# neherlab/pangraph

Measured on AMD Instinct MI355X. Metric: aligned Gbp/s in `pangraph build` (bases handed to the aligner per second, all merges, all self-merge rounds), higher is better.
Workload: dtype u8

## Files before the change

pangraph_amd/csrc/pga_chain.hip:

```cpp
#include "pga_common.h"
#include "pga_sort_exact.h"
#include "pga_sort_wave.h"
#include "pga_wave.h"
#include "pga_pipeline.h"
#include "pga_wg_sort.h"
#include <rocprim/rocprim.hpp>
#include <cstdio>

namespace pga {

struct ChainParams {
	int32_t max_dist, max_dist_inner, bw, max_skip, cap, min_cnt, min_sc;
	float pen_gap, pen_skip;
};

struct __attribute__((aligned(16))) CNode {
	double pri;
	int32_t y;
	int32_t c[2];
	int32_t s;
	uint32_t size;
	int32_t bal;
};

// ... 158 lines not shown
		if (root < 0) return -1;
		for (p = root; p >= 0;) { c = cmp(lo_y, lo_i, p); path[0][plen[0]] = p, pc[0][plen[0]++] = (int8_t)c; if (c < 0) p = nd[p].c[0]; else if (c > 0) p = nd[p].c[1]; else break; }
		for (p = root; p >= 0;) { c = cmp(hi_y, hi_i, p); path[1][plen[1]] = p, pc[1][plen[1]++] = (int8_t)c; if (c < 0) p = nd[p].c[0]; else if (c > 0) p = nd[p].c[1]; else break; }
		for (i = 0; i < plen[0] && i < plen[1]; ++i)
			if (path[0][i] == path[1][i] && pc[0][i] <= 0 && pc[1][i] >= 0) break;
		if (i == plen[0] || i == plen[1]) return -1;
		lca = i, mn = path[0][lca];
		for (i = lca + 1; i < plen[0]; ++i) if (pc[0][i] <= 0) {
			int32_t u = path[0][i], r = nd[u].c[1];
			if (nd[u].pri < nd[mn].pri) mn = u;
			if (r >= 0 && nd[nd[r].s].pri < nd[mn].pri) mn = nd[r].s;
		}
		for (i = lca + 1; i < plen[1]; ++i) if (pc[1][i] >= 0) {
			int32_t u = path[1][i], l = nd[u].c[0];
			if (nd[u].pri < nd[mn].pri) mn = u;
			if (l >= 0 && nd[nd[l].s].pri < nd[mn].pri) mn = nd[l].s;
		}
		return mn;
	}
};

struct Iter { int32_t stack[CMAXD]; int top; };


#define CF_WI 1024
#define CF_MAXIN 256

__device__ __forceinline__ int32_t score_pair32(int32_t xi, int32_t yi, int32_t xj, int32_t yj, int32_t span_j, float pen_gap, float pen_skip, int32_t *exact, int32_t *width)
{
	const int32_t dq = yi - yj, dr = xi - xj;
	const int32_t dd = dr > dq ? dr - dq : dq - dr;
	const int32_t dg = dr < dq ? dr : dq;
	int32_t sc = span_j < dg ? span_j : dg;
	*width = dd;
	if (exact) *exact = (dd == 0 && dg <= span_j);
	if (dd || dq > span_j) {
		float lin_pen = __fadd_rn(__fmul_rn(pen_gap, (float)dd), __fmul_rn(pen_skip, (float)dg));
		float log_pen = dd >= 1 ? mg_log2((float)(dd + 1)) : 0.0f;
		sc -= (int)__fadd_rn(lin_pen, __fmul_rn(.5f, log_pen));
	}
	return sc;
}

struct __attribute__((aligned(8))) CfEnt { int32_t y, x; };
__device__ __forceinline__ double cf_pri(int32_t f, int32_t x, int32_t y, float pen_gap) { return -((double)f + 0.5 * (double)pen_gap * (double)(x + y)); }

#define CF_CLK() (PROF == 2 ? (long long)clock64() : 0LL)
template <int CF_W, int PROF>
__global__ __launch_bounds__(64)
void k_chain_fast(const u128 *__restrict__ a, const uint64_t *__restrict__ seg_start, const uint32_t *__restrict__ seg_order, uint32_t n_seg,
                  uint64_t n_total, const uint64_t *__restrict__ q_aoff, int n_seq, ChainParams P,
                  int32_t *__restrict__ f, int32_t *__restrict__ pp, uint32_t *__restrict__ seg_flag, const uint32_t *__restrict__ only_flagged, unsigned long long *__restrict__ prof)
{
	constexpr int CF_M = CF_W - 1;
	__shared__ CfEnt r_e[CF_W];
	__shared__ int32_t r_f[CF_W];
	__shared__ uint8_t s_sp[CF_W];
	__shared__ int32_t r_p[CF_WI], r_t[CF_WI];
	__shared__ int32_t s_sc[CF_WI], s_j[CF_WI];
	__shared__ uint8_t s_fl[CF_WI];
	const int lane = threadIdx.x;
	const uint32_t sidx = blockIdx.x;
	if (sidx >= n_seg) return;
	const uint32_t sg = seg_order[sidx];
	if (only_flagged && !only_flagged[sg]) return;
	const uint64_t b = seg_start[sg], e = sg + 1 < n_seg ? seg_start[sg + 1] : n_total;
	const int32_t n = (int32_t)(e - b);
	const u128 *A = a + b;
	int32_t *F = f + b, *PP = pp + b;
	int qlo = 0, qhi = n_seq;
	while (qlo < qhi) { int m = (qlo + qhi) >> 1; if (q_aoff[m + 1] <= b) qlo = m + 1; else qhi = m; }
	const bool seg_is_query_start = (q_aoff[qlo] == b);
	int32_t max_dist = P.max_dist, max_dist_inner = P.max_dist_inner;
	if (max_dist < P.bw) max_dist = P.bw;
	if (max_dist_inner <= 0 || max_dist_inner >= max_dist) max_dist_inner = 0;
	for (int k = lane; k < CF_WI; k += 64) r_t[k] = -1;
	int32_t st = 0, st_in = 0, i0 = 0;
	bool bail = false; int why = 0;
	double sm_pri = 1e300; int32_t sm_arg = -1, sm_blk = -1, sm_ymin = 0, sm_ymax = 0;
	double p_floor = 1e300, p_last = 1e300;
	const int32_t FS_NONE = -(1 << 30);
	int32_t fs_floor = FS_NONE, fs_last = FS_NONE, sm_fs = FS_NONE;
	const bool shortcut_ok = P.cap >= CF_W;
	const unsigned long long c0 = wall_clock64();
	unsigned long long n_scan = 0, n_inner = 0, n_incand = 0, n_slow = 0, n_pev = 0, n_py = 0;
	unsigned long long n_stretch = 0, n_chunk = 0, n_skipstop = 0, n_sum = 0, n_sumscan = 0;
	long long tk_scan = 0, tk_red = 0, tk_best = 0, tk_inner = 0, tk_store = 0;
	u128 nxtv; nxtv.x = 0, nxtv.y = 0;
	if (lane < n) nxtv = A[lane];
	for (int32_t blk = 0; blk < n && !bail; blk += 64) {
		const int32_t bx = (int32_t)nxtv.x, by = (int32_t)nxtv.y, bsp = (int32_t)(nxtv.y >> 32 & 0xff);
		int32_t bf = 0;
		if (blk + lane < n) { const int32_t s = (blk + lane) & CF_M; r_e[s].x = bx; r_e[s].y = by; s_sp[s] = (uint8_t)bsp; }
		if (blk + 64 + lane < n) nxtv = A[blk + 64 + lane];
		__builtin_amdgcn_fence(__ATOMIC_SEQ_CST, "wavefront");
		{
			const int32_t xb = __builtin_amdgcn_readlane(bx, 0);
			for (;;) {
				const int32_t j = st + lane;
				const bool keep = j >= i0 || !(xb - r_e[j & CF_M].x > max_dist);
				const unsigned long long m = __ballot(keep);
				if (m) { st += __ffsll((long long)m) - 1; break; }
				st += 64;
			}
			p_floor = wave_min_f64_key((lane < CF_W / 64 && sm_blk >= 0 && sm_blk + 64 > st) ? sm_pri : 1e300);
			fs_floor = wave_max_i32((lane < CF_W / 64 && sm_blk >= 0 && sm_blk + 64 > st) ? sm_fs : FS_NONE);
		}
		if (blk + 128 - st > CF_W) { bail = true; why = 1; break; }
		const int32_t blk_end = blk + 64 < n ? blk + 64 : n;
		for (int32_t i = blk; i < blk_end; ++i) {
			const int il = i - blk;
			const int32_t xi = __builtin_amdgcn_readlane(bx, il), yi = __builtin_amdgcn_readlane(by, il), q_span = __builtin_amdgcn_readlane(bsp, il);
			int32_t max_f = q_span, max_j = -1;
			if (shortcut_ok && il > 0 && i0 == i - 1 && p_last < p_floor) {
				const int32_t xpl = wave_shr1(bx, 0), ypl = wave_shr1(by, 0), spl = wave_shr1(bsp, 0);
				const int32_t dr = bx - xpl, dq = by - ypl;
				const int32_t f_l = __builtin_amdgcn_readlane(bf, il - 1) + (bx - __builtin_amdgcn_readlane(bx, il - 1));
				const bool c_ok = lane >= il && blk + lane < blk_end && dr > 0 && dr <= max_dist && dq == dr && dr <= spl && dr < max_dist && f_l > bsp;
				const unsigned long long m2 = __ballot(c_ok) >> il;
				const int R = ~m2 ? __ffsll((long long)~m2) - 1 : 64;
				if (R >= 2) {
					if (lane >= il && lane < il + R) { bf = f_l; r_f[(blk + lane) & CF_M] = f_l; r_p[(blk + lane) & (CF_WI - 1)] = blk + lane - 1; }
					__builtin_amdgcn_fence(__ATOMIC_SEQ_CST, "wavefront");
					const int la = il + R - 2, lb = il + R - 1;
					p_floor = cf_pri(__builtin_amdgcn_readlane(bf, la), __builtin_amdgcn_readlane(bx, la), __builtin_amdgcn_readlane(by, la), P.pen_gap);
					p_last = cf_pri(__builtin_amdgcn_readlane(bf, lb), __builtin_amdgcn_readlane(bx, lb), __builtin_amdgcn_readlane(by, lb), P.pen_gap);
					{
						const int32_t fsm = wave_max_i32((lane >= il && lane < il + R - 1) ? bf + bsp : FS_NONE);
						fs_floor = max(max(fs_floor, fs_last), fsm);
						fs_last = __builtin_amdgcn_readlane(bf, lb) + __builtin_amdgcn_readlane(bsp, lb);
					}
					if (PROF) { n_py += R; n_stretch += R; }
					i0 = i + R - 1;
					i += R - 1;
					continue;
				}
			}
			long long k0 = CF_CLK(), k1 = k0, k2 = k0;
			int32_t best_j = -1;
			bool shortcut = false;
			if (shortcut_ok && il > 0 && i0 == i - 1) {
				const int32_t xp = __builtin_amdgcn_readlane(bx, il - 1), yp = __builtin_amdgcn_readlane(by, il - 1);
				if (xp != xi && xi - xp <= max_dist && yp < yi && yp > yi - max_dist && p_last < p_floor) { shortcut = true; best_j = i - 1; i0 = i; if (PROF) ++n_py; }
			}
			if (il > 0 && p_last < p_floor) p_floor = p_last;
			if (!shortcut) {
			if (i0 < i) { const int32_t x0 = i0 >= blk ? __builtin_amdgcn_readlane(bx, i0 - blk) : r_e[i0 & CF_M].x; if (x0 != xi) i0 = i; }
			k0 = CF_CLK();
			for (;;) {
				const int32_t j = st + lane;
				const bool keep = j >= i0 || !(xi - r_e[j & CF_M].x > max_dist);
				const unsigned long long m = __ballot(keep);
				if (m) { st += __ffsll((long long)m) - 1; break; }
				st += 64;
			}
			double best = 1e300; bool tie = false;
			{
				const int32_t y_lo = yi - max_dist;
				auto scan64 = [&](int32_t j0, int32_t jend) {
					++n_scan;
					const int32_t j = j0 + lane;
					if (j >= st && j < jend) {
						const CfEnt ej = r_e[j & CF_M];
						const bool in = ej.y > y_lo && (ej.y < yi || (ej.y == yi && seg_is_query_start && j == 0));
						if (in) { const double pj = cf_pri(r_f[j & CF_M], ej.x, ej.y, P.pen_gap); if (pj < best) best = pj, best_j = j, tie = false; else if (pj == best) tie = true; }
					}
				};
				const int32_t S = blk < (i0 & ~63) ? blk : (i0 & ~63);
				bool part = false, took = false;
				if (lane < CF_W / 64 && sm_blk >= 0 && sm_blk + 64 > st && sm_blk + 64 <= S) {
					const bool none = sm_ymax <= y_lo || sm_ymin > yi || (sm_ymin == yi && !(seg_is_query_start && sm_blk == 0));
					if ((sm_blk >= st || sm_arg >= st) && sm_ymin > y_lo && sm_ymax < yi) { best = sm_pri; best_j = sm_arg < 0 ? sm_blk : sm_arg; tie = sm_arg < 0; took = true; }
					else if (!none) part = true;
				}
				unsigned long long pm = __ballot(part);
				if (PROF) { n_sum += __popcll(__ballot(took)); n_sumscan += __popcll(pm); }
				while (pm) {
					const int bsel = __ffsll((long long)pm) - 1;
					pm &= pm - 1;
					const int32_t bb = __builtin_amdgcn_readlane(sm_blk, bsel);
					scan64(bb, bb + 64);
				}
				if (i0 > blk) {
					++n_scan;
					const int32_t j = blk + lane;
					if (j >= st && j < i0) {
						const bool in = by > y_lo && (by < yi || (by == yi && seg_is_query_start && j == 0));
						if (in) { const double pj = cf_pri(bf, bx, by, P.pen_gap); if (pj < best) best = pj, best_j = j, tie = false; else if (pj == best) tie = true; }
					}
				} else for (int32_t tj = S > st ? S : st; tj < i0; tj += 64) scan64(tj, i0);
			}
			if (i0 - st > P.cap) { bail = true; why = 2; break; }
			k1 = CF_CLK();
			{
				const unsigned long long bits = (unsigned long long)__double_as_longlong(best);
				const unsigned long long key = (bits >> 63) ? ~bits : (bits | 0x8000000000000000ULL);
				const uint32_t khi = (uint32_t)(key >> 32), klo = (uint32_t)key;
				const uint32_t mhi = wave_min_u32(khi);
				const uint32_t mlo = wave_min_u32(khi == mhi ? klo : 0xffffffffu);
				const bool is_min = khi == mhi && klo == mlo;
				const unsigned long long who = __ballot(best_j >= 0 && is_min);
				if (who == 0) best_j = -1;
				else {
					if (__popcll(who) > 1 || __ballot(tie && is_min)) { bail = true; why = 3; break; }
					best_j = __builtin_amdgcn_readlane(best_j, __ffsll((long long)who) - 1);
				}
			}
			}
			k2 = CF_CLK();
			long long k3 = k2;
			if (best_j >= 0) {
				int32_t exact, width; const int32_t j = best_j;
				CfEnt ej; int32_t fj, spj;
				if (j >= blk) { const int jl = j - blk; ej.x = __builtin_amdgcn_readlane(bx, jl); ej.y = __builtin_amdgcn_readlane(by, jl); fj = __builtin_amdgcn_readlane(bf, jl); spj = __builtin_amdgcn_readlane(bsp, jl); }
				else { ej = r_e[j & CF_M]; fj = r_f[j & CF_M]; spj = s_sp[j & CF_M]; }
				int32_t sc = fj + score_pair32(xi, yi, ej.x, ej.y, spj, P.pen_gap, P.pen_skip, &exact, &width);
				if (width <= P.bw && sc > max_f) max_f = sc, max_j = j;
				k3 = CF_CLK();
				if (!exact && (j == i - 1 ? fs_floor : max(fs_floor, fs_last)) <= max_f) { exact = 1; if (PROF) ++n_pev; }
				if (!exact && max_dist_inner > 0 && yi > 0) {
					if (st_in < st) st_in = st;
					{
						const int32_t lo = i0 - (CF_MAXIN + 1);
						if (lo > st_in && xi - r_e[lo & CF_M].x > max_dist_inner) st_in = lo + 1;
					}
					for (;;) {
						const int32_t jj = st_in + lane;
						const bool keep = jj >= i0 || !(xi - r_e[jj & CF_M].x > max_dist_inner);
						const unsigned long long m = __ballot(keep);
						if (m) { st_in += __ffsll((long long)m) - 1; break; }
						st_in += 64;
					}
					if (st_in > i0) st_in = i0;
				}
				if (!exact && max_dist_inner > 0 && st_in < i0 && yi > 0) {
					const int32_t n_in = i0 - st_in;
					if (n_in > CF_WI) { bail = true; why = 4; break; }
					if (n_in > CF_MAXIN) {
						++n_inner; n_incand += n_in; if (PROF) ++n_chunk;
						auto cand = [&](int32_t jc, int32_t &sc, bool &ok) -> bool {
							const CfEnt ec = r_e[jc & CF_M];
							if (!(ec.y <= yi - 1 && ec.y >= yi - max_dist_inner)) { sc = 0; ok = false; return false; }
							int32_t wdt;
							sc = r_f[jc & CF_M] + score_pair32(xi, yi, ec.x, ec.y, s_sp[jc & CF_M], P.pen_gap, P.pen_skip, nullptr, &wdt);
							ok = wdt <= P.bw;
							return true;
						};
						bool unsorted = false;
						for (int32_t c0 = 0; c0 < n_in; c0 += 64) {
							const int32_t jc = i0 - 1 - (c0 + lane);
							if (jc >= st_in) {
								if (jc + 1 < i0 && r_e[(jc + 1) & CF_M].y < r_e[jc & CF_M].y) unsorted = true;
								int32_t sc; bool ok;
								if (cand(jc, sc, ok) && ok) { const int32_t pj = r_p[jc & (CF_WI - 1)]; if (pj >= st_in) r_t[pj & (CF_WI - 1)] = i; }
							}
						}
						__builtin_amdgcn_fence(__ATOMIC_SEQ_CST, "wavefront");
						const bool uns = __ballot(unsorted) != 0;
						int32_t n_slots = n_in;
						if (uns) {
							++n_slow;
							n_slots = 0;
							for (int32_t c0 = 0; c0 < n_in; c0 += 64) {
								const int32_t jc = i0 - 1 - (c0 + lane);
								int32_t sc = 0; bool ok = false;
								const bool val = jc >= st_in && cand(jc, sc, ok);
								n_slots += __popcll(__ballot(val));
								if (val) {
									const int32_t yc = r_e[jc & CF_M].y;
									int32_t rank = 0;
									for (int32_t jo = st_in; jo < i0; ++jo) {
										const int32_t yo = r_e[jo & CF_M].y;
										const bool vo = yo <= yi - 1 && yo >= yi - max_dist_inner;
										rank += (vo && (yo > yc || (yo == yc && jo > jc))) ? 1 : 0;
									}
									s_sc[rank] = sc; s_j[rank] = jc;
									s_fl[rank] = (uint8_t)((ok ? 1 : 0) | (r_t[jc & (CF_WI - 1)] == i ? 2 : 0));
								}
							}
							__builtin_amdgcn_fence(__ATOMIC_SEQ_CST, "wavefront");
						}
						int32_t n_skip = 0; bool stop = false;
						for (int32_t c0 = 0; c0 < n_slots && !stop; c0 += 64) {
							int32_t v_sc = 0, v_j = -1; bool v_ok = false, v_mk = false;
							if (uns) {
								const int32_t c = c0 + lane;
								if (c < n_slots) { const int32_t fl = s_fl[c]; v_ok = fl & 1; v_mk = (fl & 2) != 0; v_sc = s_sc[c]; v_j = s_j[c]; }
							} else {
								const int32_t jc = i0 - 1 - (c0 + lane);
								if (jc >= st_in) { v_j = jc; const bool val = cand(jc, v_sc, v_ok); v_mk = val && r_t[jc & (CF_WI - 1)] == i; }
							}
							const int32_t v = v_ok ? v_sc : INT32_MIN;
							const int32_t incl = wave_prefix_max_incl(v);
							int32_t excl = __builtin_amdgcn_update_dpp(max_f, incl, 0x138, 0xf, 0xf, false);
							if (excl < max_f) excl = max_f;
							const bool is_max = v_ok && v_sc > excl;
							const unsigned long long mx = __ballot(is_max), inc = __ballot(v_ok && !is_max && v_mk);
							unsigned long long rest = mx; int last = -1, pos = 0;
							for (;;) {
								const int c = rest ? __ffsll((long long)rest) - 1 : 64;
								const unsigned long long range = (c >= 64 ? ~0ULL : ((1ULL << c) - 1)) & ~((1ULL << pos) - 1);
								n_skip += __popcll(inc & range);
// ... 18 lines not shown
						if (jc >= st_in) {
							const CfEnt ec = r_e[jc & CF_M];
							if (jc + 1 < i0 && r_e[(jc + 1) & CF_M].y < ec.y) unsorted = true;
							if (ec.y <= yi - 1 && ec.y >= yi - max_dist_inner) {
								int32_t wdt;
								c_val[k] = true;
								c_sc[k] = r_f[jc & CF_M] + score_pair32(xi, yi, ec.x, ec.y, s_sp[jc & CF_M], P.pen_gap, P.pen_skip, nullptr, &wdt);
								c_ok[k] = wdt <= P.bw;
								if (c_ok[k]) { const int32_t pj = r_p[jc & (CF_WI - 1)]; if (pj >= st_in) r_t[pj & (CF_WI - 1)] = i; }
							}
						}
					}
					__builtin_amdgcn_fence(__ATOMIC_SEQ_CST, "wavefront");
#pragma unroll
					for (int k = 0; k < CF_MAXIN / 64; ++k) if (64 * k < n_in) c_mk[k] = c_val[k] && r_t[c_j[k] & (CF_WI - 1)] == i;
					if (__ballot(unsorted)) {
						++n_slow;
						int32_t n_valid = 0;
#pragma unroll
						for (int k = 0; k < CF_MAXIN / 64; ++k) n_valid += __popcll(__ballot(c_val[k]));
#pragma unroll
						for (int k = 0; k < CF_MAXIN / 64; ++k) {
							if (c_val[k]) {
								const int32_t jc = c_j[k], yc = r_e[jc & CF_M].y;
								int32_t rank = 0;
#pragma unroll 8
								for (int32_t jo = st_in; jo < i0; ++jo) {
									const int32_t yo = r_e[jo & CF_M].y;
									const bool vo = yo <= yi - 1 && yo >= yi - max_dist_inner;
									rank += (vo && (yo > yc || (yo == yc && jo > jc))) ? 1 : 0;
								}
								s_sc[rank] = c_sc[k]; s_j[rank] = jc;
								s_fl[rank] = (uint8_t)((c_ok[k] ? 1 : 0) | (c_mk[k] ? 2 : 0));
							}
						}
						__builtin_amdgcn_fence(__ATOMIC_SEQ_CST, "wavefront");
#pragma unroll
						for (int k = 0; k < CF_MAXIN / 64; ++k) {
							const int32_t c = lane + 64 * k;
							c_val[k] = c < n_valid; c_ok[k] = false; c_mk[k] = false;
							if (c_val[k]) { const int32_t fl = s_fl[c]; c_ok[k] = fl & 1; c_mk[k] = (fl & 2) != 0; c_sc[k] = s_sc[c]; c_j[k] = s_j[c]; }
						}
						__builtin_amdgcn_fence(__ATOMIC_SEQ_CST, "wavefront");
					}
					int32_t n_skip = 0; bool stop = false;
#pragma unroll
					for (int k = 0; k < CF_MAXIN / 64; ++k) {
						if (stop || 64 * k >= n_in) break;
						const int32_t v = c_ok[k] ? c_sc[k] : INT32_MIN;
						const int32_t incl = wave_prefix_max_incl(v);
						int32_t excl = __builtin_amdgcn_update_dpp(max_f, incl, 0x138, 0xf, 0xf, false);
						if (excl < max_f) excl = max_f;
						const bool is_max = c_ok[k] && c_sc[k] > excl;
						const unsigned long long mx = __ballot(is_max), inc = __ballot(c_ok[k] && !is_max && c_mk[k]);
						unsigned long long rest = mx; int last = -1, pos = 0;
						for (;;) {
							const int c = rest ? __ffsll((long long)rest) - 1 : 64;
							const unsigned long long range = (c >= 64 ? ~0ULL : ((1ULL << c) - 1)) & ~((1ULL << pos) - 1);
							n_skip += __popcll(inc & range);
							if (n_skip > P.max_skip) { stop = true; if (PROF) ++n_skipstop; break; }
							if (c >= 64) break;
							rest &= rest - 1;
							last = c; if (n_skip > 0) --n_skip;
							pos = c + 1;
							if (pos >= 64) break;
						}
						if (last >= 0) { max_f = __builtin_amdgcn_readlane(c_sc[k], last); max_j = __builtin_amdgcn_readlane(c_j[k], last); }
					}
					}
				}
			}
			const long long k4 = CF_CLK();
			if (lane == il) bf = max_f;
			p_last = cf_pri(max_f, xi, yi, P.pen_gap);
			fs_floor = max(fs_floor, fs_last); fs_last = max_f + q_span;
			if (lane == 0) {
				r_f[i & CF_M] = max_f; r_p[i & (CF_WI - 1)] = max_j;
			}
			__builtin_amdgcn_fence(__ATOMIC_SEQ_CST, "wavefront");
			const long long k5 = CF_CLK();
			tk_scan += k1 - k0; tk_red += k2 - k1; tk_best += k3 - k2; tk_inner += k4 - k3; tk_store += k5 - k4;
		}
		if (bail) break;
		if (blk + lane < n) { F[blk + lane] = bf; PP[blk + lane] = r_p[(blk + lane) & (CF_WI - 1)]; }
		if (blk + 64 <= n) {
			CfEnt eb; eb.x = bx, eb.y = by;
			const double pb = cf_pri(bf, eb.x, eb.y, P.pen_gap);
			const double mp = wave_min_f64(pb);
			const unsigned long long who = __ballot(pb == mp);
			const int32_t ymin = wave_min_i32(eb.y), ymax = wave_max_i32(eb.y), fsb = wave_max_i32(bf + bsp);
			if (lane == ((blk >> 6) & (CF_W / 64 - 1))) {
				sm_fs = fsb;
				sm_pri = mp; sm_arg = __popcll(who) == 1 ? blk + (int32_t)(__ffsll((long long)who) - 1) : -1;
				sm_blk = blk; sm_ymin = ymin; sm_ymax = ymax;
			}
		}
	}
	if (lane == 0) seg_flag[sg] = bail ? (uint32_t)(why ? why : 1) : 0u;
	if (PROF && prof && lane == 0) {
		const unsigned long long dt = wall_clock64() - c0;
		atomicAdd(&prof[0], dt); atomicMax(&prof[1], dt); atomicMax(&prof[2], (unsigned long long)n);
		atomicAdd(&prof[12], n_pev); atomicAdd(&prof[13], n_py);
		atomicAdd(&prof[16], n_stretch); atomicAdd(&prof[17], n_chunk); atomicAdd(&prof[18], n_skipstop); atomicAdd(&prof[19], n_sum); atomicAdd(&prof[20], n_sumscan);
		atomicAdd(&prof[3], n_scan); atomicAdd(&prof[4], n_inner); atomicAdd(&prof[5], n_incand); atomicAdd(&prof[6], n_slow);
		atomicAdd(&prof[7], (unsigned long long)tk_scan); atomicAdd(&prof[8], (unsigned long long)tk_red); atomicAdd(&prof[9], (unsigned long long)tk_best); atomicAdd(&prof[10], (unsigned long long)tk_inner); atomicAdd(&prof[11], (unsigned long long)tk_store);
	}
}
#undef CF_CLK

__global__ void k_chain_segments(const u128 *__restrict__ a, const uint64_t *__restrict__ seg_start, const uint32_t *__restrict__ seg_order, uint32_t n_seg,
                                 uint64_t n_total, const uint64_t *__restrict__ q_aoff, int n_seq, const uint32_t *__restrict__ seg_flag,
                                 ChainParams P, CNode *__restrict__ nd_main, CNode *__restrict__ nd_inner,
                                 int32_t *__restrict__ f, int32_t *__restrict__ pp, int32_t *__restrict__ t)
{
	uint32_t sidx = blockIdx.x * blockDim.x + threadIdx.x;
	if (sidx >= n_seg) return;
	const uint32_t sg = seg_order[sidx];
	if (seg_flag && !seg_flag[sg]) return;
	const uint64_t b = seg_start[sg], e = sg + 1 < n_seg ? seg_start[sg + 1] : n_total;
	int qlo = 0, qhi = n_seq;
	while (qlo < qhi) { int m = (qlo + qhi) >> 1; if (q_aoff[m + 1] <= b) qlo = m + 1; else qhi = m; }
	const int32_t hi_i = -(int32_t)(b - q_aoff[qlo]);
	const int32_t n = (int32_t)(e - b);
	const u128 *A = a + b;
	int32_t *F = f + b, *PP = pp + b, *T = t + b;
	Tree<true> Tm; Tm.nd = nd_main + b; Tm.root = -1;
	Tree<false> Ti; Ti.nd = nd_inner + b; Ti.root = -1;
	int32_t max_dist = P.max_dist, max_dist_inner = P.max_dist_inner;
	if (max_dist < P.bw) max_dist = P.bw;
	if (max_dist_inner <= 0 || max_dist_inner >= max_dist) max_dist_inner = 0;
	int32_t st = 0, st_inner = 0, i0 = 0;
	for (int32_t i = 0; i < n; ++i) {
		const u128 ai = A[i];
		int32_t max_j = -1, q_span = (int32_t)(ai.y >> 32 & 0xff), max_f = q_span;
		if (i0 < i && A[i0].x != ai.x) {
			for (int32_t j = i0; j < i; ++j) {
				const u128 aj = A[j];
				const double pri = -((double)F[j] + 0.5 * (double)P.pen_gap * (double)((int32_t)aj.x + (int32_t)aj.y));
				Tm.nd[j].y = (int32_t)aj.y, Tm.nd[j].pri = pri;
				Tm.insert(j);
				if (max_dist_inner > 0) { Ti.nd[j].y = (int32_t)aj.y; Ti.insert(j); }
			}
			i0 = i;
		}
		while (st < i && (ai.x >> 32 != A[st].x >> 32 || ai.x > A[st].x + (uint64_t)max_dist || (int32_t)Tm.sz(Tm.root) > P.cap)) {
			if (st < i0) Tm.erase(st);
			++st;
		}
		if (max_dist_inner > 0) {
			while (st_inner < i && (ai.x >> 32 != A[st_inner].x >> 32 || ai.x > A[st_inner].x + (uint64_t)max_dist_inner || (int32_t)Ti.sz(Ti.root) > P.cap)) {
				if (st_inner < i0) Ti.erase(st_inner);
				++st_inner;
			}
		}
		const int32_t yi = (int32_t)ai.y;
		int32_t q = Tm.rmq(yi - max_dist, INT32_MAX, yi, hi_i);
		if (q >= 0) {
			int32_t sc, exact, width, n_skip = 0, j = q;
			sc = F[j] + score_pair(ai, A[j], P.pen_gap, P.pen_skip, &exact, &width);
			if (width <= P.bw && sc > max_f) max_f = sc, max_j = j;
			if (!exact && Ti.root >= 0 && yi > 0) {
				Iter it; int32_t p = Ti.root, lower = -1;
				while (p >= 0) { if (yi - 1 < Ti.nd[p].y) p = Ti.nd[p].c[0]; else lower = p, p = Ti.nd[p].c[1]; }
				if (lower >= 0) {
					it.top = -1;
					for (p = Ti.root; p >= 0;) { int c = Ti.cmp(Ti.nd[lower].y, lower, p); it.stack[++it.top] = p; if (c < 0) p = Ti.nd[p].c[0]; else if (c > 0) p = Ti.nd[p].c[1]; else break; }
					for (;;) {
						const int32_t ej = it.stack[it.top];
						if (Ti.nd[ej].y < yi - max_dist_inner) break;
						j = ej;
						sc = F[j] + score_pair(ai, A[j], P.pen_gap, P.pen_skip, nullptr, &width);
						if (width <= P.bw) {
							if (sc > max_f) { max_f = sc, max_j = j; if (n_skip > 0) --n_skip; }
							else if (T[j] == i) { if (++n_skip > P.max_skip) break; }
							if (PP[j] >= 0) T[PP[j]] = i;
						}
						p = Ti.nd[it.stack[it.top]].c[0];
						if (p >= 0) { for (; p >= 0; p = Ti.nd[p].c[1]) it.stack[++it.top] = p; }
						else {
							do { p = it.stack[it.top--]; } while (it.top >= 0 && p == Ti.nd[it.stack[it.top]].c[0]);
							if (it.top < 0) break;
						}
					}
				}
			}
		}
		F[i] = max_f, PP[i] = max_j;
	}
// ... 281 lines not shown
	const int q = blockIdx.x;
	if (q >= n_sub) return;
	const uint64_t s = src_off[q], d = dst_off[q], n = dst_off[q + 1] - d;
	for (uint64_t i = (uint64_t)blockIdx.y * blockDim.x + threadIdx.x; i < n; i += (uint64_t)gridDim.y * blockDim.x) out[d + i] = a[s + i];
}

static std::mutex g_chain_routes_mu;
static int64_t g_chain_routes[CHAIN_N_ROUTES];
void chain_routes_take(int64_t out[CHAIN_N_ROUTES])
{
	std::lock_guard<std::mutex> lk(g_chain_routes_mu);
	for (int i = 0; i < CHAIN_N_ROUTES; ++i) { out[i] = g_chain_routes[i]; g_chain_routes[i] = 0; }
}

static void chain_core(const DBuf<u128> &a, const DBuf<uint64_t> &q_aoff, const int n_seq, uint64_t n_a, const mm_mapopt_t &opt, int k, ChainResult &O, hipStream_t st, Timers *tm,
                       bool spec, const uint32_t *d_q_tie_x, std::vector<uint32_t> *need_out, ChainTap *tap = nullptr)
{
	if (need_out) need_out->assign((size_t)n_seq, 0u);
	if (tap) { tap->f.clear(); tap->p.clear(); tap->ev.assign((size_t)n_seq, 0u); }
	const bool counting = tap && tap->count;
	O.n_u.assign((size_t)n_seq, 0); O.n_v.assign((size_t)n_seq, 0); O.u.clear(); O.a.clear(); O.d_a.release();
	if (n_a == 0) return;
	if (n_a >= (1ULL << 31)) throw std::runtime_error("pga: more than 2^31 anchors in one batch");
	ChainParams P;
	P.max_dist = opt.max_gap, P.max_dist_inner = opt.rmq_inner_dist, P.bw = opt.bw, P.max_skip = opt.max_chain_skip, P.cap = opt.rmq_size_cap;
	P.min_cnt = opt.min_cnt, P.min_sc = opt.min_chain_score;
	P.pen_gap = (float)(opt.chain_gap_scale * 0.01 * k);
	P.pen_skip = (float)(opt.chain_skip_scale * 0.01 * k);
	int32_t seg_dist = P.max_dist < P.bw ? P.bw : P.max_dist;
	const unsigned nba = (unsigned)((n_a + 255) / 256);
	const bool vmarks = getenv("PGA_VERBOSE") != nullptr;
	auto wall = [] { return std::chrono::duration<double>(std::chrono::steady_clock::now().time_since_epoch()).count(); };
	double t_mark = vmarks ? wall() : 0.0; std::string marks;
	auto mark = [&](const char *what) { if (!vmarks) return; (void)sync_stream(st); const double t = wall(); char b[96]; snprintf(b, sizeof b, " %s %.1f", what, (t - t_mark) * 1e3); marks += b; t_mark = t; };
	DBuf<uint32_t> flag(n_a + 1); flag.zero(st);
	hipLaunchKernelGGL(k_mark_query_starts, dim3((unsigned)((n_seq + 255) / 256)), dim3(256), 0, st, q_aoff.p, n_seq, n_a, flag.p);
	hipLaunchKernelGGL(k_seg_flags, dim3(nba), dim3(256), 0, st, a.p, n_a, seg_dist, flag.p);
	DBuf<uint64_t> pos(n_a + 1);
	{
		size_t tb = 0;
		auto it = rocprim::make_transform_iterator(flag.p, [] __device__ (uint32_t v) { return (uint64_t)v; });
		PGA_HIP(rocprim::exclusive_scan(nullptr, tb, it, pos.p, (uint64_t)0, n_a + 1, rocprim::plus<uint64_t>(), st));
		DBuf<uint8_t> tmp(tb ? tb : 1);
		PGA_HIP(rocprim::exclusive_scan(tmp.p, tb, it, pos.p, (uint64_t)0, n_a + 1, rocprim::plus<uint64_t>(), st));
	}
	uint64_t n_seg64 = 0;
	PGA_HIP(hipMemcpyAsync(&n_seg64, pos.p + n_a, 8, hipMemcpyDeviceToHost, st));
	PGA_HIP(sync_stream(st));
	const uint32_t n_seg = (uint32_t)n_seg64;
	DBuf<uint64_t> seg_start(n_seg);
	hipLaunchKernelGGL(k_seg_starts, dim3(nba), dim3(256), 0, st, flag.p, pos.p, n_a, seg_start.p);
	DBuf<uint32_t> seg_incl(n_a);
	{
		struct Op { const uint32_t *flag; const uint64_t *pos; uint32_t *out; };
		Op op{flag.p, pos.p, seg_incl.p};
		PGA_HIP(rocprim::transform(rocprim::make_counting_iterator<uint64_t>(0), rocprim::make_discard_iterator(), n_a,
		        [op] __device__ (uint64_t i) { op.out[i] = (uint32_t)(op.pos[i] + op.flag[i]); return 0; }, st));
	}
	DBuf<uint32_t> neg_len(n_seg), ord0(n_seg), neg_len2(n_seg), ord(n_seg);
	hipLaunchKernelGGL(k_seg_len, dim3((n_seg + 255) / 256), dim3(256), 0, st, seg_start.p, n_seg, n_a, neg_len.p, ord0.p);
	static const bool wg_sort = !(getenv("PGA_WG_SORT") && getenv("PGA_WG_SORT")[0] == '0');
	if (wg_sort && n_seg > 0 && n_seg <= WGS_CAP)
		hipLaunchKernelGGL((k_wg_sort_pairs<uint32_t>), dim3(1), dim3(WGS_NT), 0, st, neg_len.p, neg_len2.p, ord0.p, ord.p, n_seg, 32);
	else {
		size_t tb = 0;
		PGA_HIP(rocprim::radix_sort_pairs(nullptr, tb, neg_len.p, neg_len2.p, ord0.p, ord.p, n_seg, 0, 32, st));
		DBuf<uint8_t> tmp(tb ? tb : 1);
		PGA_HIP(rocprim::radix_sort_pairs(tmp.p, tb, neg_len.p, neg_len2.p, ord0.p, ord.p, n_seg, 0, 32, st));
	}
	mark("segments");
	DBuf<CNode> nd_main, nd_inner;
	DBuf<uint32_t> seg_q;
	DBuf<int32_t> f(n_a), pp(n_a), t(n_a), v(n_a);
	t.zero(st);
	mark("buffers");
	{
		DBuf<uint32_t> seg_flag(n_seg);
		seg_q.alloc((size_t)n_seq); seg_q.zero(st);
		EventTimer et(st);
		const bool use_fast = !getenv("PGA_CHAIN_EXACT_ONLY");
		if (!use_fast && n_seq > 0) PGA_HIP(hipMemsetD32Async((hipDeviceptr_t)seg_q.p, 1, (size_t)n_seq, st));
		const bool verbose = getenv("PGA_VERBOSE") != nullptr;
		const bool prof_on = verbose && getenv("PGA_CHAIN_PROF");
		DBuf<unsigned long long> cprof(32); if (prof_on || counting) cprof.zero(st);
		if (use_fast && prof_on) hipLaunchKernelGGL((k_chain_fast<2048, 2>), dim3(n_seg), dim3(64), 0, st, a.p, seg_start.p, ord.p, n_seg, n_a, q_aoff.p, n_seq, P, f.p, pp.p, seg_flag.p, (const uint32_t*)nullptr, cprof.p);
		else if (use_fast && counting) hipLaunchKernelGGL((k_chain_fast<2048, 1>), dim3(n_seg), dim3(64), 0, st, a.p, seg_start.p, ord.p, n_seg, n_a, q_aoff.p, n_seq, P, f.p, pp.p, seg_flag.p, (const uint32_t*)nullptr, cprof.p);
		else if (use_fast) {
			hipLaunchKernelGGL((k_chain_fast<2048, 0>), dim3(n_seg), dim3(64), 0, st, a.p, seg_start.p, ord.p, n_seg, n_a, q_aoff.p, n_seq, P, f.p, pp.p, seg_flag.p, (const uint32_t*)nullptr, (unsigned long long*)nullptr);
		}
		const double ms_fast = verbose ? et.stop() : 0.0;
		bool any_flagged = !use_fast;
		if (use_fast) {
			DBuf<uint32_t> n_fl(1);
			struct Fl { const uint32_t *f; };
			Fl fl{seg_flag.p};
			auto it = rocprim::make_transform_iterator(rocprim::make_counting_iterator<uint32_t>(0), [fl] __device__ (uint32_t i) { return (uint32_t)(fl.f[i] != 0); });
			size_t tb = 0;
			PGA_HIP(rocprim::reduce(nullptr, tb, it, n_fl.p, 0u, (size_t)n_seg, rocprim::plus<uint32_t>(), st));
			DBuf<uint8_t> tmp(tb ? tb : 1);
			PGA_HIP(rocprim::reduce(tmp.p, tb, it, n_fl.p, 0u, (size_t)n_seg, rocprim::plus<uint32_t>(), st));
			any_flagged = n_fl.download(st)[0] != 0;
		}
		if (any_flagged) {
			if (use_fast) hipLaunchKernelGGL(k_seg_query_flag, dim3((n_seg + 255) / 256), dim3(256), 0, st, seg_flag.p, seg_start.p, n_seg, q_aoff.p, n_seq, seg_q.p);
			nd_main.alloc(n_a); nd_inner.alloc(n_a);
			hipLaunchKernelGGL(k_chain_segments, dim3((n_seg + 63) / 64), dim3(64), 0, st, a.p, seg_start.p, ord.p, n_seg, n_a, q_aoff.p, n_seq,
			                   use_fast ? seg_flag.p : (const uint32_t*)nullptr, P, nd_main.p, nd_inner.p, f.p, pp.p, t.p);
		}
		PGA_HIP(hipGetLastError());
		const double ms = et.stop(K_CHAIN);
		if (getenv("PGA_VERBOSE") && use_fast) {
			std::vector<uint32_t> fl = seg_flag.download(st); size_t nf = 0, why[5] = {0, 0, 0, 0, 0}; for (uint32_t v : fl) { nf += v != 0; ++why[v < 5 ? v : 1]; }
			fprintf(stderr, "[pga]   chain: %u segments, %zu re-run by the tree kernel (ring overflow %zu, size cap %zu, tied minimum %zu, inner candidates %zu), %.3f ms (fast kernel %.3f ms)\n", n_seg, nf, why[1], why[2], why[3], why[4], ms, ms_fast);
			if (nf) { std::vector<uint64_t> ss = seg_start.download(st); for (uint32_t s = 0; s < n_seg; ++s) if (fl[s]) fprintf(stderr, "[pga]     segment %u: %llu anchors, reason %u\n", s, (unsigned long long)((s + 1 < n_seg ? ss[s + 1] : n_a) - ss[s]), fl[s]); }
			std::vector<unsigned long long> pr = cprof.download(st);
			if (prof_on) fprintf(stderr, "[pga]   chain fast: longest segment %llu anchors, slowest %.2f ms, sum %.1f ms; scan iterations %.2f/anchor, inner scans %.3f/anchor with %.1f candidates, %llu unsorted\n",
			        pr[2], pr[1] * 1e-5, pr[0] * 1e-5, (double)pr[3] / (double)n_a, (double)pr[4] / (double)n_a, pr[4] ? (double)pr[5] / (double)pr[4] : 0.0, pr[6]);
			if (prof_on) fprintf(stderr, "[pga]   chain fast clocks/anchor: scan %.0f reduce %.0f best %.0f inner %.0f store %.0f; inner scans skipped by the f + span bound %.3f/anchor; shortcut taken %.3f\n", (double)pr[7] / n_a, (double)pr[8] / n_a, (double)pr[9] / n_a, (double)pr[10] / n_a, (double)pr[11] / n_a, (double)pr[12] / n_a, (double)pr[13] / n_a);
		}
		if (tm) { tm->kern[K_CHAIN].ms += ms; tm->kern[K_CHAIN].launches += 1; tm->kern[K_CHAIN].alg_bytes += 36.0 * (double)n_a; }
		if (counting && use_fast) {
			const std::vector<uint32_t> fl = seg_flag.download(st);
			const std::vector<unsigned long long> pr = cprof.download(st);
			std::lock_guard<std::mutex> lk(g_chain_routes_mu);
			int64_t *R = g_chain_routes;
			for (uint32_t v : fl) ++R[v == 0 ? CR_FAST : CR_WHY1 + (int)((v < 5 ? v : 1) - 1)];
			R[CR_STRETCH] += (int64_t)pr[16]; R[CR_SINGLE] += (int64_t)(pr[13] - pr[16]); R[CR_BOUND] += (int64_t)pr[12];
			R[CR_INNER_REG] += (int64_t)(pr[4] - pr[17]); R[CR_INNER_CHUNK] += (int64_t)pr[17]; R[CR_RERANK] += (int64_t)pr[6]; R[CR_SKIP_STOP] += (int64_t)pr[18];
			R[CR_SUMMARY] += (int64_t)pr[19]; R[CR_SUMMARY_SCAN] += (int64_t)pr[20];
		}
	}
	hipLaunchKernelGGL(k_fix_pred, dim3(nba), dim3(256), 0, st, seg_start.p, n_seg, n_a, q_aoff.p, n_seq, seg_incl.p, pp.p);
	if (tap) { tap->f = f.download(st); tap->p = pp.download(st); }
	mark("chain kernels");
	DBuf<u128> z(n_a), w(n_a), out(n_a);
	DBuf<uint64_t> u(n_a), u2(n_a);
	DBuf<int32_t> n_u((size_t)n_seq), n_v((size_t)n_seq);
	{
		EventTimer et(st);
		const bool verbose = getenv("PGA_VERBOSE") != nullptr;
		DBuf<unsigned long long> prof(16); if (verbose || counting) prof.zero(st);
		DBuf<int64_t> n_z((size_t)n_seq);
		DBuf<uint32_t> ev((size_t)n_seq), q_tie_f;
		hipLaunchKernelGGL(k_bt_list, dim3((unsigned)n_seq), dim3(64), 0, st, n_seq, q_aoff.p, f.p, t.p, z.p, P, n_z.p, n_u.p, n_v.p);
		double ms_list = 0, ms_sort = 0;
		et.mark();
		EventTimer et2(st);
		static const bool z_hint = getenv("PGA_NO_Z_HINT") == nullptr;
		if (!z_hint && !spec) replay_sort_segments(z.p, n_a, q_aoff.p, n_z.p, n_seq, nullptr, st, tm);
		else {
			DBuf<uint64_t> key0(n_a), key1(n_a), sx(n_a), sy(n_a);
			DBuf<uint32_t> idx0(n_a), idx1(n_a), dupc(n_a);
			DBuf<uint32_t> &q_tie = q_tie_f; q_tie.alloc((size_t)n_seq);
			q_tie.zero(st);
			hipLaunchKernelGGL(k_z_keys, dim3(nba), dim3(256), 0, st, z.p, q_aoff.p, n_z.p, n_seq, n_a, key0.p, idx0.p);
			int bits = 1; while ((1LL << bits) < n_seq) ++bits;
			if (wg_sort && n_a <= WGS_CAP)
				hipLaunchKernelGGL((k_wg_sort_pairs<uint64_t>), dim3(1), dim3(WGS_NT), 0, st, key0.p, key1.p, idx0.p, idx1.p, (uint32_t)n_a, 32 + bits);
			else {
			size_t tb = 0;
			PGA_HIP(rocprim::radix_sort_pairs(nullptr, tb, key0.p, key1.p, idx0.p, idx1.p, n_a, 0, 32 + bits, st));
			DBuf<uint8_t> tmp(tb ? tb : 1);
			PGA_HIP(rocprim::radix_sort_pairs(tmp.p, tb, key0.p, key1.p, idx0.p, idx1.p, n_a, 0, 32 + bits, st));
			}
			hipLaunchKernelGGL(k_z_sorted, dim3(nba), dim3(256), 0, st, z.p, key1.p, idx1.p, n_a, q_aoff.p, n_z.p, sx.p, sy.p, q_tie.p);
			{
				struct Dp { const uint64_t *k; };
				Dp dp{key1.p};
				auto flag_it = rocprim::make_transform_iterator(rocprim::make_counting_iterator<uint64_t>(0), [dp] __device__ (uint64_t i) { return (uint32_t)(i > 0 && dp.k[i] == dp.k[i - 1]); });
				size_t tb2 = 0;
				PGA_HIP(rocprim::inclusive_scan(nullptr, tb2, flag_it, dupc.p, n_a, rocprim::plus<uint32_t>(), st));
				DBuf<uint8_t> tmp2(tb2 ? tb2 : 1);
				PGA_HIP(rocprim::inclusive_scan(tmp2.p, tb2, flag_it, dupc.p, n_a, rocprim::plus<uint32_t>(), st));
			}
			hipLaunchKernelGGL(k_z_take_sorted, dim3(nba), dim3(256), 0, st, z.p, sx.p, sy.p, q_aoff.p, n_z.p, n_seq, spec ? (const uint32_t*)nullptr : q_tie.p, n_a);
			const RsHint hint{sx.p, sy.p, dupc.p};
			if (!spec) { replay_sort_segments(z.p, n_a, q_aoff.p, n_z.p, n_seq, q_tie.p, st, tm, &hint); PGA_HIP(sync_stream(st)); }
		}
		et2.mark();
		EventTimer et3(st);
		hipLaunchKernelGGL(k_bt_walk, dim3((unsigned)n_seq), dim3(64), 0, st, n_seq, q_aoff.p, a.p, f.p, pp.p, t.p, v.p, z.p, n_z.p, u.p, w.p, u2.p, out.p, P, n_u.p, n_v.p,
		                   verbose || counting ? prof.p : (unsigned long long*)nullptr, ev.p);
		if (n_a) hipLaunchKernelGGL(k_bt_copy, dim3((unsigned)((n_a + 255) / 256)), dim3(256), 0, st, n_seq, q_aoff.p, (uint64_t)n_a, a.p, v.p, u.p, w.p, n_u.p, n_v.p, out.p);
		const double ms_walk = et3.stop(K_BACKTRACK);
		ms_list = et.finish(K_BACKTRACK); ms_sort = et2.finish();
		if (verbose) {
			std::vector<uint32_t> he = ev.download(st), hq = q_tie_f.n ? q_tie_f.download(st) : std::vector<uint32_t>();
			size_t c[4] = {0, 0, 0, 0}, ft = 0; for (size_t i = 0; i < he.size(); ++i) { c[0] += he[i] & 1; c[1] += (he[i] >> 1) & 1; c[2] += (he[i] >> 2) & 1; c[3] += he[i] != 0; ft += i < hq.size() && hq[i]; }
			fprintf(stderr, "[pga]   backtrack order events: %zu of %d queries (%zu with equal scores): walk stopped at an equal-score mark %zu, candidate marked by an equal score %zu, equal chain starts %zu\n", c[3], n_seq, ft, c[0], c[1], c[2]);
		}
		if (tap) tap->ev = ev.download(st);
		if (counting) { const std::vector<unsigned long long> pr = prof.download(st); std::lock_guard<std::mutex> lk(g_chain_routes_mu); g_chain_routes[CR_BT_RELOAD] += (int64_t)pr[13]; }
		if (spec && need_out) {
			DBuf<uint32_t> need((size_t)n_seq);
			hipLaunchKernelGGL(k_need_exact, dim3((unsigned)((n_seq + 255) / 256)), dim3(256), 0, st, n_seq, d_q_tie_x, q_tie_f.p, ev.p, seg_q.p, need.p);
			*need_out = need.download(st);
		}
		const double ms = ms_list + ms_walk;
		if (verbose) {
			std::vector<unsigned long long> pr = prof.download(st);
			fprintf(stderr, "[pga]   backtrack: %.3f ms = candidate lists %.3f + walks %.3f; sort replay %.3f (per-query max: walks %.2f, compact %.2f ms)\n", ms, ms_list, ms_walk, ms_sort,
// ... 83 lines not shown
```

Measured before the change: 8.057.

## Rebuild chain score floors lazily and carry block-boundary anchor across blocks

The fast chaining kernel no longer recomputes the priority and f+span floors with two wave reductions at every 64-anchor block. It rebuilds them lazily, only when a shortcut or the bound check fails on the stale floors. It also carries the last anchor of the previous block (x, y, span, f) in registers and keeps per-block summaries that exclude lane 63. This lets the stretch shortcut and the single-predecessor shortcut fire at lane 0 across block boundaries, where previously they were skipped. Extra profiling counters and clocks are added, which adds bookkeeping and some risk of subtle correctness differences in the floor logic.

```diff
diff --git a/pangraph_amd/csrc/pga_chain.hip b/pangraph_amd/csrc/pga_chain.hip
--- a/pangraph_amd/csrc/pga_chain.hip
+++ b/pangraph_amd/csrc/pga_chain.hip
@@ -264,13 +264,20 @@
 	const int32_t FS_NONE = -(1 << 30);
 	int32_t fs_floor = FS_NONE, fs_last = FS_NONE, sm_fs = FS_NONE;
 	const bool shortcut_ok = P.cap >= CF_W;
+	int32_t c_x = 0, c_y = 0, c_sp = 0, c_f = 0;
+	double sm_pri63 = 1e300; int32_t sm_fs63 = FS_NONE;
+	int32_t st_blk = 0; bool fresh = false;
 	const unsigned long long c0 = wall_clock64();
 	unsigned long long n_scan = 0, n_inner = 0, n_incand = 0, n_slow = 0, n_pev = 0, n_py = 0;
 	unsigned long long n_stretch = 0, n_chunk = 0, n_skipstop = 0, n_sum = 0, n_sumscan = 0;
+	unsigned long long n_rebuild = 0;
 	long long tk_scan = 0, tk_red = 0, tk_best = 0, tk_inner = 0, tk_store = 0;
+	long long tk_pro = 0, tk_sum = 0, tk_str = 0, tk_try = 0;
+	const long long k_all = CF_CLK();
 	u128 nxtv; nxtv.x = 0, nxtv.y = 0;
 	if (lane < n) nxtv = A[lane];
 	for (int32_t blk = 0; blk < n && !bail; blk += 64) {
+		const long long kb0 = CF_CLK();
 		const int32_t bx = (int32_t)nxtv.x, by = (int32_t)nxtv.y, bsp = (int32_t)(nxtv.y >> 32 & 0xff);
 		int32_t bf = 0;
 		if (blk + lane < n) { const int32_t s = (blk + lane) & CF_M; r_e[s].x = bx; r_e[s].y = by; s_sp[s] = (uint8_t)bsp; }
@@ -285,19 +292,37 @@
 				if (m) { st += __ffsll((long long)m) - 1; break; }
 				st += 64;
 			}
-			p_floor = wave_min_f64_key((lane < CF_W / 64 && sm_blk >= 0 && sm_blk + 64 > st) ? sm_pri : 1e300);
-			fs_floor = wave_max_i32((lane < CF_W / 64 && sm_blk >= 0 && sm_blk + 64 > st) ? sm_fs : FS_NONE);
-		}
+			st_blk = st; fresh = false;
+		}
+		auto rebuild_floors = [&](int il) {
+			const bool live = lane < CF_W / 64 && sm_blk >= 0 && sm_blk + 64 > st_blk;
+			const bool edge = il == 0 && sm_blk == blk - 64;
+			double pv = live ? (edge ? sm_pri63 : sm_pri) : 1e300;
+			int32_t fv = live ? (edge ? sm_fs63 : sm_fs) : FS_NONE;
+			if (lane < il - 1) { const double pl = cf_pri(bf, bx, by, P.pen_gap); pv = pl < pv ? pl : pv; fv = max(fv, bf + bsp); }
+			p_floor = wave_min_f64_key(pv);
+			fs_floor = wave_max_i32(fv);
+			fresh = true;
+			if (PROF) ++n_rebuild;
+		};
 		if (blk + 128 - st > CF_W) { bail = true; why = 1; break; }
 		const int32_t blk_end = blk + 64 < n ? blk + 64 : n;
+		tk_pro += CF_CLK() - kb0;
 		for (int32_t i = blk; i < blk_end; ++i) {
 			const int il = i - blk;
 			const int32_t xi = __builtin_amdgcn_readlane(bx, il), yi = __builtin_amdgcn_readlane(by, il), q_span = __builtin_amdgcn_readlane(bsp, il);
 			int32_t max_f = q_span, max_j = -1;
-			if (shortcut_ok && il > 0 && i0 == i - 1 && p_last < p_floor) {
-				const int32_t xpl = wave_shr1(bx, 0), ypl = wave_shr1(by, 0), spl = wave_shr1(bsp, 0);
+			const long long ks = CF_CLK();
+			bool floor_ok = false;
+			if (shortcut_ok && i0 == i - 1) {
+				floor_ok = p_last < p_floor;
+				if (!floor_ok && !fresh) { rebuild_floors(il); floor_ok = p_last < p_floor; }
+			}
+			const int32_t xp = il > 0 ? __builtin_amdgcn_readlane(bx, il - 1) : c_x, yp = il > 0 ? __builtin_amdgcn_readlane(by, il - 1) : c_y;
+			if (floor_ok) {
+				const int32_t xpl = wave_shr1(bx, c_x), ypl = wave_shr1(by, c_y), spl = wave_shr1(bsp, c_sp);
 				const int32_t dr = bx - xpl, dq = by - ypl;
-				const int32_t f_l = __builtin_amdgcn_readlane(bf, il - 1) + (bx - __builtin_amdgcn_readlane(bx, il - 1));
+				const int32_t f_l = (il > 0 ? __builtin_amdgcn_readlane(bf, il - 1) : c_f) + (bx - xp);
 				const bool c_ok = lane >= il && blk + lane < blk_end && dr > 0 && dr <= max_dist && dq == dr && dr <= spl && dr < max_dist && f_l > bsp;
 				const unsigned long long m2 = __ballot(c_ok) >> il;
 				const int R = ~m2 ? __ffsll((long long)~m2) - 1 : 64;
@@ -315,17 +340,16 @@
 					if (PROF) { n_py += R; n_stretch += R; }
 					i0 = i + R - 1;
 					i += R - 1;
+					tk_str += CF_CLK() - ks;
 					continue;
 				}
 			}
 			long long k0 = CF_CLK(), k1 = k0, k2 = k0;
+			tk_try += k0 - ks;
 			int32_t best_j = -1;
 			bool shortcut = false;
-			if (shortcut_ok && il > 0 && i0 == i - 1) {
-				const int32_t xp = __builtin_amdgcn_readlane(bx, il - 1), yp = __builtin_amdgcn_readlane(by, il - 1);
-				if (xp != xi && xi - xp <= max_dist && yp < yi && yp > yi - max_dist && p_last < p_floor) { shortcut = true; best_j = i - 1; i0 = i; if (PROF) ++n_py; }
-			}
-			if (il > 0 && p_last < p_floor) p_floor = p_last;
+			if (floor_ok && xp != xi && xi - xp <= max_dist && yp < yi && yp > yi - max_dist) { shortcut = true; best_j = i - 1; i0 = i; if (PROF) ++n_py; }
+			if (p_last < p_floor) p_floor = p_last;
 			if (!shortcut) {
 			if (i0 < i) { const int32_t x0 = i0 >= blk ? __builtin_amdgcn_readlane(bx, i0 - blk) : r_e[i0 & CF_M].x; if (x0 != xi) i0 = i; }
 			k0 = CF_CLK();
@@ -395,11 +419,20 @@
 				int32_t exact, width; const int32_t j = best_j;
 				CfEnt ej; int32_t fj, spj;
 				if (j >= blk) { const int jl = j - blk; ej.x = __builtin_amdgcn_readlane(bx, jl); ej.y = __builtin_amdgcn_readlane(by, jl); fj = __builtin_amdgcn_readlane(bf, jl); spj = __builtin_amdgcn_readlane(bsp, jl); }
+				else if (j == blk - 1) { ej.x = c_x; ej.y = c_y; fj = c_f; spj = c_sp; }
 				else { ej = r_e[j & CF_M]; fj = r_f[j & CF_M]; spj = s_sp[j & CF_M]; }
 				int32_t sc = fj + score_pair32(xi, yi, ej.x, ej.y, spj, P.pen_gap, P.pen_skip, &exact, &width);
 				if (width <= P.bw && sc > max_f) max_f = sc, max_j = j;
 				k3 = CF_CLK();
-				if (!exact && (j == i - 1 ? fs_floor : max(fs_floor, fs_last)) <= max_f) { exact = 1; if (PROF) ++n_pev; }
+				if (!exact) {
+					int32_t fs_rest = j == i - 1 ? fs_floor : max(fs_floor, fs_last);
+					if (fs_rest > max_f && !fresh) {
+						rebuild_floors(il);
+						if (p_last < p_floor) p_floor = p_last;
+						fs_rest = j == i - 1 ? fs_floor : max(fs_floor, fs_last);
+					}
+					if (fs_rest <= max_f) { exact = 1; if (PROF) ++n_pev; }
+				}
 				if (!exact && max_dist_inner > 0 && yi > 0) {
 					if (st_in < st) st_in = st;
 					{
@@ -584,19 +617,25 @@
 			tk_scan += k1 - k0; tk_red += k2 - k1; tk_best += k3 - k2; tk_inner += k4 - k3; tk_store += k5 - k4;
 		}
 		if (bail) break;
+		const long long kb1 = CF_CLK();
 		if (blk + lane < n) { F[blk + lane] = bf; PP[blk + lane] = r_p[(blk + lane) & (CF_WI - 1)]; }
 		if (blk + 64 <= n) {
 			CfEnt eb; eb.x = bx, eb.y = by;
 			const double pb = cf_pri(bf, eb.x, eb.y, P.pen_gap);
-			const double mp = wave_min_f64(pb);
+			const long long pb_bits = __double_as_longlong(pb);
+			const double p63 = __longlong_as_double(((long long)__builtin_amdgcn_readlane((int)(pb_bits >> 32), 63) << 32) | (unsigned)__builtin_amdgcn_readlane((int)(pb_bits & 0xffffffffLL), 63));
+			const int32_t fs63 = __builtin_amdgcn_readlane(bf + bsp, 63);
+			const double mp63 = wave_min_f64(lane < 63 ? pb : 1e300), mp = p63 < mp63 ? p63 : mp63;
 			const unsigned long long who = __ballot(pb == mp);
-			const int32_t ymin = wave_min_i32(eb.y), ymax = wave_max_i32(eb.y), fsb = wave_max_i32(bf + bsp);
+			const int32_t ymin = wave_min_i32(eb.y), ymax = wave_max_i32(eb.y), fsb63 = wave_max_i32(lane < 63 ? bf + bsp : FS_NONE);
 			if (lane == ((blk >> 6) & (CF_W / 64 - 1))) {
-				sm_fs = fsb;
-				sm_pri = mp; sm_arg = __popcll(who) == 1 ? blk + (int32_t)(__ffsll((long long)who) - 1) : -1;
+				sm_fs = max(fsb63, fs63); sm_fs63 = fsb63;
+				sm_pri = mp; sm_pri63 = mp63; sm_arg = __popcll(who) == 1 ? blk + (int32_t)(__ffsll((long long)who) - 1) : -1;
 				sm_blk = blk; sm_ymin = ymin; sm_ymax = ymax;
 			}
-		}
+			c_x = __builtin_amdgcn_readlane(bx, 63); c_y = __builtin_amdgcn_readlane(by, 63); c_sp = __builtin_amdgcn_readlane(bsp, 63); c_f = __builtin_amdgcn_readlane(bf, 63);
+		}
+		tk_sum += CF_CLK() - kb1;
 	}
 	if (lane == 0) seg_flag[sg] = bail ? (uint32_t)(why ? why : 1) : 0u;
 	if (PROF && prof && lane == 0) {
@@ -606,6 +645,13 @@
 		atomicAdd(&prof[16], n_stretch); atomicAdd(&prof[17], n_chunk); atomicAdd(&prof[18], n_skipstop); atomicAdd(&prof[19], n_sum); atomicAdd(&prof[20], n_sumscan);
 		atomicAdd(&prof[3], n_scan); atomicAdd(&prof[4], n_inner); atomicAdd(&prof[5], n_incand); atomicAdd(&prof[6], n_slow);
 		atomicAdd(&prof[7], (unsigned long long)tk_scan); atomicAdd(&prof[8], (unsigned long long)tk_red); atomicAdd(&prof[9], (unsigned long long)tk_best); atomicAdd(&prof[10], (unsigned long long)tk_inner); atomicAdd(&prof[11], (unsigned long long)tk_store);
+		if (PROF == 2 && sidx == 0) {
+			prof[46] = n_rebuild;
+			const unsigned long long v[14] = {(unsigned long long)n, n_stretch, n_py, (unsigned long long)tk_scan, (unsigned long long)tk_red, (unsigned long long)tk_best, (unsigned long long)tk_inner,
+			                                  (unsigned long long)tk_store, (unsigned long long)tk_pro, (unsigned long long)tk_sum, (unsigned long long)tk_str, (unsigned long long)tk_try,
+			                                  (unsigned long long)(CF_CLK() - k_all), n_scan};
+			for (int k = 0; k < 14; ++k) prof[32 + k] = v[k];
+		}
 	}
 }
 #undef CF_CLK
@@ -1053,7 +1099,7 @@
 		if (!use_fast && n_seq > 0) PGA_HIP(hipMemsetD32Async((hipDeviceptr_t)seg_q.p, 1, (size_t)n_seq, st));
 		const bool verbose = getenv("PGA_VERBOSE") != nullptr;
 		const bool prof_on = verbose && getenv("PGA_CHAIN_PROF");
-		DBuf<unsigned long long> cprof(32); if (prof_on || counting) cprof.zero(st);
+		DBuf<unsigned long long> cprof(64); if (prof_on || counting) cprof.zero(st);
 		if (use_fast && prof_on) hipLaunchKernelGGL((k_chain_fast<2048, 2>), dim3(n_seg), dim3(64), 0, st, a.p, seg_start.p, ord.p, n_seg, n_a, q_aoff.p, n_seq, P, f.p, pp.p, seg_flag.p, (const uint32_t*)nullptr, cprof.p);
 		else if (use_fast && counting) hipLaunchKernelGGL((k_chain_fast<2048, 1>), dim3(n_seg), dim3(64), 0, st, a.p, seg_start.p, ord.p, n_seg, n_a, q_aoff.p, n_seq, P, f.p, pp.p, seg_flag.p, (const uint32_t*)nullptr, cprof.p);
 		else if (use_fast) {
@@ -1088,6 +1134,9 @@
 			if (prof_on) fprintf(stderr, "[pga]   chain fast: longest segment %llu anchors, slowest %.2f ms, sum %.1f ms; scan iterations %.2f/anchor, inner scans %.3f/anchor with %.1f candidates, %llu unsorted\n",
 			        pr[2], pr[1] * 1e-5, pr[0] * 1e-5, (double)pr[3] / (double)n_a, (double)pr[4] / (double)n_a, pr[4] ? (double)pr[5] / (double)pr[4] : 0.0, pr[6]);
 			if (prof_on) fprintf(stderr, "[pga]   chain fast clocks/anchor: scan %.0f reduce %.0f best %.0f inner %.0f store %.0f; inner scans skipped by the f + span bound %.3f/anchor; shortcut taken %.3f\n", (double)pr[7] / n_a, (double)pr[8] / n_a, (double)pr[9] / n_a, (double)pr[10] / n_a, (double)pr[11] / n_a, (double)pr[12] / n_a, (double)pr[13] / n_a);
+			if (prof_on) fprintf(stderr, "[pga]   chain fast, longest segment: %llu anchors, %llu by the stretch, %llu by the single shortcut, %llu by the full path (%llu scan iterations, floors rebuilt %llu times); clocks: all %llu = scan %llu reduce %llu best %llu inner %llu store %llu"
+			        " + block prologue %llu block epilogue %llu stretches written %llu stretches tried in vain %llu + rest %lld\n", pr[32], pr[33], pr[34] - pr[33], pr[32] - pr[34], pr[45], pr[46], pr[44], pr[35], pr[36], pr[37], pr[38], pr[39],
+			        pr[40], pr[41], pr[42], pr[43], (long long)pr[44] - (long long)(pr[35] + pr[36] + pr[37] + pr[38] + pr[39] + pr[40] + pr[41] + pr[42] + pr[43]));
 		}
 		if (tm) { tm->kern[K_CHAIN].ms += ms; tm->kern[K_CHAIN].launches += 1; tm->kern[K_CHAIN].alg_bytes += 36.0 * (double)n_a; }
 		if (counting && use_fast) {
```

New measurement: 8.328, median of 5. 1.03x the previous value.
